# danielbulhosa/CURL

Measured on AMD Instinct MI355X. Metric: Mpix/s through fused curve-apply at 1500x1000 bs32; PSNR delta vs ref, higher is better.
Workload: dtype f32; 1 GPU; CURLLayer.forward fused 3-stage (RGB->Lab->RGB->HSV->RGB + residual), bool mask all ones (every pixel computed); batch_per_gpu=32, global_batch=32, height=1000, width=1500, knots=randn*0.1 (160 per image), parallelism=image-sharded x1, no data-path collective, clock_settle_launches=150

## Files before the change

### curl_amd/csrc/curl_math.h

```cpp
#pragma once
#include <math.h>
#include <type_traits>

#if defined(__HIPCC__)
#define CURL_HD __host__ __device__ __forceinline__
#else
#define CURL_HD inline
#endif

namespace curlm {

CURL_HD float hw_log2(float x) {
#if defined(__HIP_DEVICE_COMPILE__)
  return __builtin_amdgcn_logf(x);
#else
  return log2f(x);
#endif
}
CURL_HD float hw_exp2(float x) {
#if defined(__HIP_DEVICE_COMPILE__)
  return __builtin_amdgcn_exp2f(x);
#else
  return exp2f(x);
#endif
// ... 150 lines not shown
}
template <int M>
CURL_HD void mul_run(float (&y)[M], const float (&a)[M], const float (&b)[M]) {
  for (int i = 0; i < M; ++i) y[i] = a[i] * b[i];
}
template <int M>
CURL_HD void scale_run(float (&y)[M], const float (&a)[M], float k) {
  for (int i = 0; i < M; ++i) y[i] = a[i] * k;
}
template <int M>
CURL_HD void rsub_run(float (&y)[M], float k, const float (&a)[M]) {
  for (int i = 0; i < M; ++i) y[i] = k - a[i];
}
#if defined(__HIP_DEVICE_COMPILE__)
__device__ __forceinline__ float select_le_hw(float x, float thr, float a, float b) {
  unsigned long long m;
  float r;
  asm("v_cmp_le_f32_e64 %0, %1, %2" : "=s"(m) : "v"(x), "s"(thr));
  asm("v_cndmask_b32_e64 %0, %1, %2, %3" : "=v"(r) : "v"(b), "v"(a), "s"(m));
  return r;
}
__device__ __forceinline__ float zero_if_less_hw(float c, float mx, float val) {
  unsigned long long m;
  float r;
  asm("v_cmp_lt_f32_e64 %0, %1, %2" : "=s"(m) : "v"(c), "v"(mx));
  asm("v_cndmask_b32_e64 %0, %1, 0, %2" : "=v"(r) : "v"(val), "s"(m));
  return r;
}
#endif

template <int M>
CURL_HD void select_le_run(float (&out)[M], const float (&x)[M], float thr, const float (&a)[M], const float (&b)[M]) {
#if defined(__HIP_DEVICE_COMPILE__)
#pragma unroll
  for (int i = 0; i < M; ++i) out[i] = select_le_hw(x[i], thr, a[i], b[i]);
  return;
#endif
  float d[M];
  rsub_run(d, thr, x);
#pragma unroll
  for (int i = 0; i < M; ++i) out[i] = blend(neg_mask(d[i]), b[i], a[i]);
}

#if defined(__HIP_DEVICE_COMPILE__)
__device__ __forceinline__ void pred_mul(float& dst, unsigned long long m, float x, float k_uniform) {
  unsigned long long t;
  asm("s_and_saveexec_b64 %1, %2\n\tv_mul_f32_e32 %0, %4, %3\n\ts_mov_b64 exec, %1"
      : "+v"(dst), "=&s"(t) : "s"(m), "v"(x), "s"(k_uniform) : "scc");
}
__device__ __forceinline__ void pred_mul_clamp(float& dst, unsigned long long m, float x, float k_uniform) {
  unsigned long long t;
  asm("s_and_saveexec_b64 %1, %2\n\tv_mul_f32_e64 %0, %4, %3 clamp\n\ts_mov_b64 exec, %1"
      : "+v"(dst), "=&s"(t) : "s"(m), "v"(x), "s"(k_uniform) : "scc");
}
__device__ __forceinline__ void pred_fma(float& dst, unsigned long long m, float x, float k_uniform, float c_vgpr) {
  unsigned long long t;
  asm("s_and_saveexec_b64 %1, %2\n\tv_fma_f32 %0, %3, %4, %5\n\ts_mov_b64 exec, %1"
      : "+v"(dst), "=&s"(t) : "s"(m), "v"(x), "s"(k_uniform), "v"(c_vgpr) : "scc");
}
template <bool BRANCH = true, int M, class A>
__device__ __forceinline__ void select_le_lazy(float (&out)[M], const float (&x)[M], float thr, A a, const float (&b)[M]) {
  unsigned long long m[M], any = BRANCH ? 0ull : 1ull;
#pragma unroll
  for (int i = 0; i < M; ++i) {
    asm("v_cmp_le_f32_e64 %0, %1, %2" : "=s"(m[i]) : "v"(x[i]), "s"(thr));
    if (BRANCH) any |= m[i];
  }
  float r[M];
#pragma unroll
  for (int i = 0; i < M; ++i) r[i] = b[i];
  if (any) {
    if constexpr (std::is_invocable_v<A, float (&)[M], const unsigned long long (&)[M]>) {
      a(r, m);
    } else {
      float av[M];
      a(av);
#pragma unroll
      for (int i = 0; i < M; ++i) asm("v_cndmask_b32_e64 %0, %0, %1, %2" : "+v"(r[i]) : "v"(av[i]), "s"(m[i]));
    }
  }
#pragma unroll
  for (int i = 0; i < M; ++i) out[i] = r[i];
}
#endif

template <int M>
CURL_HD void pow_run(float (&x)[M], float e) {
  CURL_FENCE();
  CURL_TRANS_BEGIN();
#pragma unroll
  for (int i = 0; i < M; ++i) x[i] = hw_log2(x[i]);
  CURL_FENCE();
  scale_run(x, x, e);
  CURL_TRANS_BEGIN();
  CURL_FENCE();
#pragma unroll
  for (int i = 0; i < M; ++i) x[i] = hw_exp2(x[i]);
  CURL_TRANS_END();
  CURL_FENCE();
}

template <int N>
CURL_HD void mat_row(float (&y)[N], const float (&a)[3 * N], float m0, float m1, float m2) {
  for (int i = 0; i < N; ++i) y[i] = fmaf(m2, a[2 * N + i], fmaf(m1, a[N + i], m0 * a[i]));
}

template <int N, int LAZY = 0>
CURL_HD void rgb2lab_n(PxN<N>& p) {
  float x[3 * N], g[3 * N], u2[3 * N], lin[3 * N];
#pragma unroll
  for (int i = 0; i < N; ++i) {
    x[i] = p.c0[i];
    x[N + i] = p.c1[i];
    x[2 * N + i] = p.c2[i];
  }
  fma_run(g, x, kInv1055, (float)(0.055 / 1.055));
  {
    mul_run(u2, g, g);
    pow_run(g, kGammaFrac);
    mul_run(g, u2, g);
  }
#if defined(__HIP_DEVICE_COMPILE__)
  if constexpr (LAZY != 0) {
    const float (&xr)[3 * N] = x;
    select_le_lazy<LAZY == 1>(x, x, kSrgbThr, [&](float (&r)[3 * N], const unsigned long long (&m)[3 * N]) {
#pragma unroll
      for (int i = 0; i < 3 * N; ++i) pred_mul(r[i], m[i], xr[i], kInv1292);
    }, g);
  } else
#endif
  {
    scale_run(lin, x, kInv1292);
    select_le_run(x, x, kSrgbThr, lin, g);
  }
  float t[3 * N], f[3 * N];
  {
    float tx[N], ty[N], tz[N];
    mat_row<N>(tx, x, 0.412453f * kInvXn, 0.357580f * kInvXn, 0.180423f * kInvXn);
    mat_row<N>(ty, x, 0.212671f, 0.715160f, 0.072169f);
    mat_row<N>(tz, x, 0.019334f * kInvZn, 0.119193f * kInvZn, 0.950227f * kInvZn);
#pragma unroll
    for (int i = 0; i < N; ++i) t[i] = tx[i], t[N + i] = ty[i], t[2 * N + i] = tz[i];
  }
#pragma unroll
  for (int i = 0; i < 3 * N; ++i) f[i] = t[i];
  pow_run(f, kThird);
#if defined(__HIP_DEVICE_COMPILE__)
  if constexpr (LAZY != 0) {
    const float (&tr)[3 * N] = t;
    select_le_lazy<LAZY == 1>(f, t, kEps3, [&](float (&r)[3 * N], const unsigned long long (&m)[3 * N]) {
      const float c = k4_29;
#pragma unroll
      for (int i = 0; i < 3 * N; ++i) pred_fma(r[i], m[i], tr[i], kInv3Eps2, c);
    }, f);
  } else
#endif
  {
    fma_run(lin, t, kInv3Eps2, k4_29);
    select_le_run(f, t, kEps3, lin, f);
  }
#pragma unroll
  for (int i = 0; i < N; ++i) {
    float fx = f[i], fy = f[N + i], fz = f[2 * N + i];
    p.c0[i] = fmaf(fy, 1.16f, -0.16f);
    p.c1[i] = fmaf(fx - fy, (float)(500.0 / 220.0), 0.5f);
    p.c2[i] = fmaf(fy - fz, (float)(200.0 / 220.0), 0.5f);
  }
}

template <int N, bool CLAMP12 = false, int LAZY = 0>
CURL_HD void lab2rgb_n(PxN<N>& p) {
  float X[3 * N], v[3 * N], g[3 * N], lin[3 * N];
#pragma unroll
  for (int i = 0; i < N; ++i) {
    float fy = fmaf(p.c0[i], (float)(100.0 / 116.0), (float)(16.0 / 116.0));
    float fx = fmaf(p.c1[i], (float)(220.0 / 500.0), fy - (float)(110.0 / 500.0));
    float fz = fmaf(p.c2[i], (float)(-220.0 / 200.0), fy + (float)(110.0 / 200.0));
    X[i] = fx, X[N + i] = fy, X[2 * N + i] = fz;
  }
  {
    float cub[3 * N];
    mul_run(cub, X, X);
    mul_run(cub, cub, X);
#if defined(__HIP_DEVICE_COMPILE__)
    if constexpr (LAZY != 0) {
      const float (&Xr)[3 * N] = X;
      select_le_lazy<LAZY == 1>(X, X, kEps, [&](float (&r)[3 * N], const unsigned long long (&m)[3 * N]) {
        const float c = -(k3Eps2 * k4_29);
#pragma unroll
        for (int i = 0; i < 3 * N; ++i) pred_fma(r[i], m[i], Xr[i], k3Eps2, c);
      }, cub);
    } else
#endif
    {
      fma_run(lin, X, k3Eps2, -(k3Eps2 * k4_29));
      select_le_run(X, X, kEps, lin, cub);
    }
  }
  {
    float r[N], gg[N], b[N];
    mat_row<N>(r, X, 3.2404542f * kXn, -1.5371385f, -0.4985314f * kZn);
    mat_row<N>(gg, X, -0.9692660f * kXn, 1.8760108f, 0.0415560f * kZn);
    mat_row<N>(b, X, 0.0556434f * kXn, -0.2040259f, 1.0572252f * kZn);
#pragma unroll
    for (int i = 0; i < N; ++i) v[i] = r[i], v[N + i] = gg[i], v[2 * N + i] = b[i];
  }
#pragma unroll
  for (int i = 0; i < 3 * N; ++i) g[i] = v[i];
  pow_run(g, kInvGamma);
  if (!CLAMP12) {
    fma_run(g, g, 1.055f, -0.055f);
#if defined(__HIP_DEVICE_COMPILE__)
    if constexpr (LAZY != 0) {
      const float (&vr)[3 * N] = v;
      select_le_lazy<LAZY == 1>(v, v, kLinThr, [&](float (&r)[3 * N], const unsigned long long (&m)[3 * N]) {
#pragma unroll
        for (int i = 0; i < 3 * N; ++i) pred_mul(r[i], m[i], vr[i], 12.92f);
      }, g);
    } else
#endif
    {
      scale_run(lin, v, 12.92f);
      select_le_run(v, v, kLinThr, lin, g);
    }
  } else {
    float g0[N], v0[N], l0[N], d[3 * N];
#pragma unroll
    for (int i = 0; i < N; ++i) g0[i] = g[i], v0[i] = v[i];
    fma_run(g0, g0, 1.055f, -0.055f);
    scale_run(l0, v0, 12.92f);
    rsub_run(d, kLinThr, v);
#pragma unroll
    for (int i = 0; i < N; ++i) g[i] = g0[i], lin[i] = l0[i];
#if defined(__HIP_DEVICE_COMPILE__)
    if constexpr (LAZY != 0) {
#pragma unroll
      for (int i = N; i < 3 * N; ++i) g[i] = clamp01(fmaf(g[i], 1.055f, -0.055f));
      const float (&vr)[3 * N] = v;
      select_le_lazy<LAZY == 1>(v, v, kLinThr, [&](float (&r)[3 * N], const unsigned long long (&m)[3 * N]) {
#pragma unroll
        for (int i = 0; i < N; ++i) pred_mul(r[i], m[i], vr[i], 12.92f);
#pragma unroll
        for (int i = N; i < 3 * N; ++i) pred_mul_clamp(r[i], m[i], vr[i], 12.92f);
      }, g);
    } else
#endif
    {
#pragma unroll
      for (int i = N; i < 3 * N; ++i) {
        g[i] = clamp01(fmaf(g[i], 1.055f, -0.055f));
        lin[i] = clamp01(v[i] * 12.92f);
      }
#if defined(__HIP_DEVICE_COMPILE__)
#pragma unroll
      for (int i = 0; i < 3 * N; ++i) v[i] = select_le_hw(v[i], kLinThr, lin[i], g[i]);
#else
#pragma unroll
      for (int i = 0; i < 3 * N; ++i) v[i] = blend(neg_mask(d[i]), g[i], lin[i]);
#endif
    }
  }
#pragma unroll
  for (int i = 0; i < N; ++i) {
    p.c0[i] = v[i];
    p.c1[i] = v[N + i];
    p.c2[i] = v[2 * N + i];
  }
}

template <int N, bool UNIT = false>
CURL_HD void rgb2hsv_n(PxN<N>& p) {
  float r[N], g[N], b[N], mx[N], nd[N], rdm[N];
#pragma unroll
  for (int i = 0; i < N; ++i) {
    r[i] = UNIT ? p.c0[i] : clampf(p.c0[i], kHsvFloor, 1.0f);
    g[i] = UNIT ? p.c1[i] : clampf(p.c1[i], kHsvFloor, 1.0f);
    b[i] = UNIT ? p.c2[i] : clampf(p.c2[i], kHsvFloor, 1.0f);
    mx[i] = fmaxf(r[i], fmaxf(g[i], b[i]));
    nd[i] = fminf(r[i], fminf(g[i], b[i])) - mx[i];
    rdm[i] = UNIT ? fmaf(-nd[i], mx[i], 1e-30f) : -nd[i] * mx[i];
  }
  CURL_FENCE();
  CURL_TRANS_BEGIN();
#pragma unroll
  for (int i = 0; i < N; ++i) rdm[i] = UNIT ? hw_rcp(rdm[i]) : rcp_refined(rdm[i]);
  CURL_TRANS_END();
  CURL_FENCE();
#pragma unroll
  for (int i = 0; i < N; ++i) {
    float dfi = rdm[i] * mx[i];
#if defined(__HIP_DEVICE_COMPILE__)
    float t0 = zero_if_less_hw(r[i], mx[i], (g[i] - b[i]) * dfi);
    float t1 = zero_if_less_hw(g[i], mx[i], fmaf(b[i] - r[i], dfi, 2.0f));
    float t2 = zero_if_less_hw(b[i], mx[i], fmaf(r[i] - g[i], dfi, 4.0f));
#else
    float t0 = drop_if(neg_mask(r[i] - mx[i]), (g[i] - b[i]) * dfi);
    float t1 = drop_if(neg_mask(g[i] - mx[i]), fmaf(b[i] - r[i], dfi, 2.0f));
    float t2 = drop_if(neg_mask(b[i] - mx[i]), fmaf(r[i] - g[i], dfi, 4.0f));
#endif
    int live = neg_mask(nd[i]);
    float h = keep_if(live, (t0 + t1) + t2);
    if (UNIT) h = fmaf(h, (float)(1.0 / 6.0), keep_if(neg_mask(h), 1.0f));
    else h = (h + keep_if(neg_mask(h), 6.0f)) * (float)(1.0 / 6.0);
    float s = nd[i] * (rdm[i] * nd[i]);
    if (!UNIT) s = keep_if(live, s);
    p.c0[i] = UNIT ? h : clampf(h, kHsvFloor, 1.0f);
    p.c1[i] = UNIT ? s : clampf(s, kHsvFloor, 1.0f);
    p.c2[i] = UNIT ? mx[i] : clampf(mx[i], kHsvFloor, 1.0f);
  }
}

CURL_HD Px rgb2lab(Px p) {
  PxN<1> q{{p.c0}, {p.c1}, {p.c2}};
  rgb2lab_n<1>(q);
  return Px{q.c0[0], q.c1[0], q.c2[0]};
}
CURL_HD Px lab2rgb(Px p) {
  PxN<1> q{{p.c0}, {p.c1}, {p.c2}};
  lab2rgb_n<1>(q);
  return Px{q.c0[0], q.c1[0], q.c2[0]};
}
CURL_HD Px rgb2hsv(Px p) {
// ... 99 lines not shown
#pragma clang fp contract(off)
#endif
  float sx = S * x;
  float acc0 = 0.0f, acc1 = 0.0f, acc2 = 0.0f;
  int j = 0;
  for (; j + 16 <= n_terms;) {
    for (int e = 0; e < 16; ++e, ++j) {
      float t = sx - (float)j;
      float p = sl[j] * t;
      acc0 = acc0 + p;
    }
    acc1 = acc1 + acc0;
    acc0 = 0.0f;
    if ((j & 0xF0) == 0) {
      acc2 = acc2 + acc1;
      acc1 = 0.0f;
    }
  }
  for (; j < n_terms; ++j) {
    float t = sx - (float)j;
    float p = sl[j] * t;
    acc0 = acc0 + p;
  }
  acc0 = acc0 + acc1;
  acc0 = acc0 + acc2;
  return c0 + acc0;
}

CURL_HD float scale_pwl(float x, const float* C, const float* sl, int K) {
  float sx = (float)(K - 1) * x;
  float fi = clampf(floorf(sx), 0.0f, (float)(K - 2));
  int i = (int)fi;
  float frac = clamp01(sx - fi);
  return fmaf(sl[i], frac, C[i]);
}

CURL_HD float scale_pwl_pairs(float x, const float* tab, int K) {
  float sx = (float)(K - 1) * x;
  float fi = clampf(floorf(sx), 0.0f, (float)(K - 2));
  int i = (int)fi;
  float frac = clamp01(sx - fi);
  return fmaf(tab[2 * i + 1], frac, tab[2 * i]);
}

CURL_HD float scale_exact_pairs(float x, const float* tab, int K) {
#if defined(__clang__)
#pragma clang fp contract(off)
#endif
  const int n_terms = K - 2;
  const float sx = (float)(K - 1) * x;
  float acc0 = 0.0f, acc1 = 0.0f, acc2 = 0.0f;
  int j = 0;
  for (; j + 16 <= n_terms;) {
    for (int e = 0; e < 16; ++e, ++j) {
      float t = sx - (float)j;
      float p = tab[2 * j + 1] * t;
      acc0 = acc0 + p;
    }
    acc1 = acc1 + acc0;
    acc0 = 0.0f;
    if ((j & 0xF0) == 0) {
      acc2 = acc2 + acc1;
      acc1 = 0.0f;
    }
  }
  for (; j < n_terms; ++j) {
    float t = sx - (float)j;
    float p = tab[2 * j + 1] * t;
    acc0 = acc0 + p;
  }
  acc0 = acc0 + acc1;
  acc0 = acc0 + acc2;
  return tab[0] + acc0;
}
template <int MODE>
CURL_HD float scale_tab(float x, const float* tab, int K) {
  return MODE == 1 ? scale_exact_pairs(x, tab, K) : scale_pwl_pairs(x, tab, K);
}

struct LayerCoef {
  Affine lab[3], rgb[3], hsv[4];
};

template <bool BINARY, int N, bool CLAMP12 = false>
CURL_HD void lab_stage_n(PxN<N>& p, const float (&m)[N], const Affine* k) {
  rgb2lab_n<N, 1>(p);
#pragma unroll
  for (int i = 0; i < N; ++i) {
    Px o = adjust3(Px{p.c0[i], p.c1[i], p.c2[i]}, k[0], k[1], k[2]);
    if (!BINARY) {
      o.c0 *= m[i];
      o.c1 *= m[i];
      o.c2 *= m[i];
    }
    p.c0[i] = o.c0, p.c1[i] = o.c1, p.c2[i] = o.c2;
  }
  lab2rgb_n<N, CLAMP12, 1>(p);
}
CURL_HD Px lab_stage_masked_out() { return lab2rgb(Px{0.0f, 0.0f, 0.0f}); }

template <bool BINARY, int N>
CURL_HD void hsv_stage_n(PxN<N>& p, const float (&m)[N], const Affine* k) {
  rgb2hsv_n<N>(p);
#pragma unroll
  for (int i = 0; i < N; ++i) {
    Px h = adjust_hsv4(Px{p.c0[i], p.c1[i], p.c2[i]}, k[0], k[1], k[2], k[3]);
    if (!BINARY) {
      h.c0 *= m[i];
      h.c1 *= m[i];
      h.c2 *= m[i];
    }
    Px o = hsv2rgb<BINARY>(h);
    if (BINARY) {
      o.c0 *= m[i];
      o.c1 *= m[i];
      o.c2 *= m[i];
    }
    p.c0[i] = o.c0, p.c1[i] = o.c1, p.c2[i] = o.c2;
  }
}

template <bool BINARY, int N>
CURL_HD void curl_layer_n(PxN<N>& p, const float (&m)[N], const LayerCoef& k) {
  PxN<N> in = p;
  lab_stage_n<BINARY, N, true>(p, m, k.lab);
#pragma unroll
  for (int i = 0; i < N; ++i) {
    Px o = adjust3<true>(Px{p.c0[i], p.c1[i], p.c2[i]}, k.rgb[0], k.rgb[1], k.rgb[2]);
    if (!BINARY) {
      o.c0 *= m[i];
      o.c1 *= m[i];
      o.c2 *= m[i];
    }
    p.c0[i] = o.c0, p.c1[i] = o.c1, p.c2[i] = o.c2;
  }
  rgb2hsv_n<N, BINARY>(p);
#pragma unroll
  for (int i = 0; i < N; ++i) {
    Px h = adjust_hsv4<BINARY>(Px{p.c0[i], p.c1[i], p.c2[i]}, k.hsv[0], k.hsv[1], k.hsv[2], k.hsv[3]);
    if (!BINARY) {
      h.c0 *= m[i];
      h.c1 *= m[i];
      h.c2 *= m[i];
    }
    Px res = hsv2rgb<BINARY>(h);
    p.c0[i] = clamp01(in.c0[i] + res.c0) * m[i];
    p.c1[i] = clamp01(in.c1[i] + res.c1) * m[i];
    p.c2[i] = clamp01(in.c2[i] + res.c2) * m[i];
  }
}

template <bool BINARY>
CURL_HD Px lab_stage(Px in, float m, const Affine* k) {
  PxN<1> q{{in.c0}, {in.c1}, {in.c2}};
  const float mm[1] = {m};
  lab_stage_n<BINARY, 1>(q, mm, k);
  return Px{q.c0[0], q.c1[0], q.c2[0]};
}
template <bool BINARY>
CURL_HD Px hsv_stage(Px in, float m, const Affine* k) {
  PxN<1> q{{in.c0}, {in.c1}, {in.c2}};
  const float mm[1] = {m};
  hsv_stage_n<BINARY, 1>(q, mm, k);
  return Px{q.c0[0], q.c1[0], q.c2[0]};
}
template <bool BINARY>
CURL_HD Px curl_layer(Px in, float m, const LayerCoef& k) {
  PxN<1> q{{in.c0}, {in.c1}, {in.c2}};
  const float mm[1] = {m};
  curl_layer_n<BINARY, 1>(q, mm, k);
  return Px{q.c0[0], q.c1[0], q.c2[0]};
}

}
```

### curl_amd/csrc/kernels/host_api.inc

```
static int check_img(const void* in, const void* out, int B, int H, int W) {
  if (!in || !out) return fail(CURL_E_NULL, "image pointer is NULL");
  if (B <= 0 || H <= 0 || W <= 0) return fail(CURL_E_SHAPE, "B, H, W must be positive");
  if ((uint64_t)H * (uint64_t)W > (1ull << 30)) return fail(CURL_E_SHAPE, "H*W exceeds 2^30 pixels");
  if (B > 65535) return fail(CURL_E_SHAPE, "B exceeds 65535 images per call");
  return 0;
}
static int check_coeffs_aligned(const float* coeffs, int num_coeffs) {
  if (num_coeffs == 126 && (uintptr_t)coeffs % 8) return fail(CURL_E_SHAPE, "coeffs must be 8-byte aligned (num_coeffs = 126)");
  if ((uintptr_t)coeffs % 4) return fail(CURL_E_SHAPE, "coeffs must be 4-byte aligned");
  return 0;
}
static int check_flags(unsigned flags, unsigned allowed) {
  const unsigned tune = CURL_F_TUNE_UNROLL_MASK | CURL_F_TUNE_BLOCK_MASK | CURL_F_TUNE_XCD_MASK | CURL_F_TUNE_OCC_MASK | CURL_F_TUNE_PREP_MASK | CURL_F_MASK_FIRST | CURL_F_TUNE_NO_NT | CURL_F_DIAG_NO_MEM;
  if (flags & ~(allowed | tune)) return fail(CURL_E_FLAGS, "unsupported flag bit for this entry point");
  if ((flags & CURL_F_EXACT_ORDER) && (flags & CURL_F_PWL))
    return fail(CURL_E_FLAGS, "CURL_F_EXACT_ORDER and CURL_F_PWL are exclusive");
  if (((flags & CURL_F_TUNE_PREP_MASK) >> CURL_F_TUNE_PREP_SHIFT) > 2)
    return fail(CURL_E_FLAGS, "curve-collapse placement must be 0 (library's choice), 1 (separate launch) or 2 (in the kernel)");
  return 0;
}

static bool planes_vec4(size_t HW, const void* mask, int mask_kind, const void* p0, const void* p1 = nullptr,
                        const void* p2 = nullptr, const void* p3 = nullptr) {
  bool ok = (HW % 4 == 0) && (((uintptr_t)p0 | (uintptr_t)p1 | (uintptr_t)p2 | (uintptr_t)p3) % 16 == 0);
  if (mask_kind == CURL_MASK_F32 && ((uintptr_t)mask % 16)) ok = false;
  if (mask_kind == CURL_MASK_U8 && ((uintptr_t)mask % 4)) ok = false;
  return ok;
}
#define DISPATCH_VEC_MASK(LAUNCH, aligned, mask_kind, ...)                            \
  do {                                                                                \
    if (aligned) {                                                                    \
      if ((mask_kind) == CURL_MASK_U8) LAUNCH(4, CURL_MASK_U8, ##__VA_ARGS__);        \
      else if ((mask_kind) == CURL_MASK_F32) LAUNCH(4, CURL_MASK_F32, ##__VA_ARGS__); \
      else LAUNCH(4, CURL_MASK_NONE, ##__VA_ARGS__);                                  \
    } else {                                                                          \
      if ((mask_kind) == CURL_MASK_U8) LAUNCH(1, CURL_MASK_U8, ##__VA_ARGS__);        \
      else if ((mask_kind) == CURL_MASK_F32) LAUNCH(1, CURL_MASK_F32, ##__VA_ARGS__); \
      else LAUNCH(1, CURL_MASK_NONE, ##__VA_ARGS__);                                  \
    }                                                                                 \
  } while (0)

constexpr unsigned kXcdDefault = 1;
struct Geometry {
  int xcd = 0;
  int vec;
  int unroll;
  unsigned n;
  unsigned blocks_per_image, n_blocks, n_images;
  int nt;
  unsigned threads = 256;
  unsigned units = 0, segs = 0;
  unsigned lds_cap = 0;
};
static int make_row_geometry(Geometry& g, int B, int H, int W) {
  if (g.vec == 4 && W % 4 != 0) g.vec = 1;
  g.units = (unsigned)(W / g.vec);
  unsigned best_t = 64, best_waste = ~0u;
  for (unsigned t = 64; t <= 256; t += 64) {
    unsigned segs = (g.units + t - 1) / t, waste = segs * t - g.units;
    if (waste <= best_waste) best_waste = waste, best_t = t;
  }
  g.threads = best_t;
  g.segs = (g.units + best_t - 1) / best_t;
  g.n = (unsigned)((size_t)H * W / g.vec);
  uint64_t per_image = (uint64_t)g.segs * (uint64_t)H;
  if (per_image * (uint64_t)B > 0x7fffffffull || per_image > 0x7fffffffull) return fail(CURL_E_SHAPE, "grid too large");
  g.blocks_per_image = (unsigned)per_image;
  g.n_blocks = (unsigned)(per_image * (uint64_t)B);
  return 0;
}


static unsigned lds_for_resident(unsigned k, unsigned static_bytes = 0) {
  const unsigned total = (k == 2 ? 43u : 128u / k) * 1280u;
  return total > static_bytes ? total - static_bytes : 0u;
}
template <auto Kernel>
static unsigned static_lds() {
  static const unsigned v = [] {
    hipFuncAttributes a;
    return hipFuncGetAttributes(&a, reinterpret_cast<const void*>(Kernel)) == hipSuccess ? (unsigned)a.sharedSizeBytes : 0u;
  }();
  return v;
}
constexpr unsigned kResidentMinTiles = 5632u;
constexpr unsigned kResPsnr = 3, kResEgress = 4, kResIngress = 4, kResLoss = 0, kResLossBwd = 0;
static unsigned aux_lds(unsigned k_resident, const dim3& grid, bool float4_path, unsigned static_bytes) {
  return (k_resident > 1 && float4_path && (uint64_t)grid.x * grid.y >= kResidentMinTiles) ? lds_for_resident(k_resident, static_bytes) : 0u;
}

static int make_geometry(Geometry& g, const void* p0, const void* p1, const void* pm, int mask_kind, int B, int H, int W,
                         unsigned flags, int default_unroll, size_t also_multiple_of_4 = 0) {
  size_t HW = (size_t)H * W;
  bool aligned = (HW % 4 == 0) && (also_multiple_of_4 % 4 == 0) && (((uintptr_t)p0 | (uintptr_t)p1) % 16 == 0);
  if (pm && mask_kind == CURL_MASK_F32 && ((uintptr_t)pm % 16)) aligned = false;
  if (pm && mask_kind == CURL_MASK_U8 && ((uintptr_t)pm % 4)) aligned = false;
  g.vec = aligned ? 4 : 1;
  int u = (int)((flags & CURL_F_TUNE_UNROLL_MASK) >> CURL_F_TUNE_UNROLL_SHIFT);
  if (u == 0) u = default_unroll;
  if (u != 1 && u != 2 && u != 4) return fail(CURL_E_FLAGS, "tuning unroll must be 1, 2 or 4");
  g.unroll = u;
  g.n = (unsigned)(HW / g.vec);
  const unsigned bsel = (flags & CURL_F_TUNE_BLOCK_MASK) >> CURL_F_TUNE_BLOCK_SHIFT;
  if (bsel > 2) return fail(CURL_E_FLAGS, "tuning block size must be 0 (256), 1 (128) or 2 (64 threads)");
  g.threads = 256u >> bsel;
  unsigned per_chunk = g.threads * (unsigned)u;
  g.blocks_per_image = (g.n + per_chunk - 1) / per_chunk;
  uint64_t nb = (uint64_t)g.blocks_per_image * (uint64_t)B;
  if (nb > 0x7fffffffull) return fail(CURL_E_SHAPE, "grid too large");
  g.n_blocks = (unsigned)nb;
  g.nt = (flags & CURL_F_TUNE_NO_NT) ? 0 : 1;
  g.n_images = (unsigned)B;
  unsigned xsel = (flags & CURL_F_TUNE_XCD_MASK) >> CURL_F_TUNE_XCD_SHIFT;
  if (xsel > 2) return fail(CURL_E_FLAGS, "tuning tile mapping must be 0 (default), 1 (plain) or 2 (XCD-contiguous)");
  g.xcd = (xsel ? xsel : kXcdDefault) == 2;
  const unsigned occ = (flags & CURL_F_TUNE_OCC_MASK) >> CURL_F_TUNE_OCC_SHIFT;
  g.lds_cap = occ > 1 ? lds_for_resident(occ) : 0u;
  return 0;
}

template <class Op, int VEC, int MK, bool NT>
static hipError_t launch_u(const Geometry& g, const StreamArgs& a, hipStream_t s) {
  dim3 grid(a.xcd_per ? 8u * a.xcd_per : g.blocks_per_image, g.n_images), block(g.threads);
  if constexpr (Op::kSingleTileShape) {
    hipLaunchKernelGGL((stream_kernel<Op, VEC, 1, MK, NT>), grid, block, g.lds_cap, s, a);
  } else {
    switch (g.unroll) {
      case 1:
        if constexpr (Op::kMask && MK == CURL_MASK_U8 && VEC == 4 && NT && Op::kLdsFloats == 0) {
          if (a.mask_first == 1) {
            hipLaunchKernelGGL((stream_kernel<Op, VEC, 1, MK, NT, FMT_F32CHW, true>), grid, block, g.lds_cap, s, a);
            break;
          }
        }
        hipLaunchKernelGGL((stream_kernel<Op, VEC, 1, MK, NT>), grid, block, g.lds_cap, s, a);
        break;
      case 2:
        hipLaunchKernelGGL((stream_kernel<Op, VEC, 2, MK, NT>), grid, block, g.lds_cap, s, a);
        break;
      default:
        hipLaunchKernelGGL((stream_kernel<Op, VEC, 4, MK, NT>), grid, block, g.lds_cap, s, a);
        break;
    }
  }
  return hipGetLastError();
}

template <class Op, int MK>
static hipError_t launch_v(const Geometry& g, const StreamArgs& a, hipStream_t s) {
  if (g.vec == 4) return g.nt ? launch_u<Op, 4, MK, true>(g, a, s) : launch_u<Op, 4, MK, false>(g, a, s);
  return launch_u<Op, 1, MK, false>(g, a, s);
}

static PrepArgs make_prep(const float* r0, int n0, int K0, const float* r1, int n1, int K1, const float* r2, int n2, int K2,
                          float* ws, unsigned stride, float* reg) {
  PrepArgs p;
  p.raw[0] = r0, p.raw[1] = r1, p.raw[2] = r2;
  p.ncurves[0] = n0, p.ncurves[1] = n1, p.ncurves[2] = n2;
  p.K[0] = K0, p.K[1] = K1, p.K[2] = K2;
  p.ws = ws;
  p.reg_out = reg;
  p.stride = stride;
  return p;
}
static int launch_prep(const PrepArgs& p, int B, hipStream_t s) {
  hipLaunchKernelGGL(knots_prep_kernel, dim3(B), dim3(256), 0, s, p);
  hipError_t e = hipGetLastError();
  if (e != hipSuccess) return hip_fail(e, "knots_prep_kernel");
  return 0;
}
static int run_prep(const float* r0, int n0, int K0, const float* r1, int n1, int K1, const float* r2, int n2, int K2,
                    float* ws, unsigned stride, float* reg, int B, hipStream_t s) {
  return launch_prep(make_prep(r0, n0, K0, r1, n1, K1, r2, n2, K2, ws, stride, reg), B, s);
}

struct Slab {
  int H_full = 0, row0 = 0;
};

constexpr unsigned kSelfPrepMaxTiles = 2048u;

template <class Op, int MK>
static hipError_t launch_selfprep(const Geometry& g, const StreamArgs& a, const PrepArgs& p, hipStream_t s) {
  dim3 grid(g.blocks_per_image, g.n_images), block(256);
  if (g.vec == 4) hipLaunchKernelGGL((stream_selfprep_kernel<Op, 4, MK, true>), grid, block, 0, s, a, p);
  else hipLaunchKernelGGL((stream_selfprep_kernel<Op, 1, MK, false>), grid, block, 0, s, a, p);
  return hipGetLastError();
}

template <class Op>
static int launch_stream(const float* in, float* out, const void* mask, int mask_kind, const float* coef,
                         unsigned coef_stride, int B, int H, int W, unsigned flags, hipStream_t s, const char* name,
                         int op_flag = 0, Slab slab = Slab(), const PrepArgs* prep = nullptr) {
  Geometry g;
  bool self_prep = false;
  if (prep) {
    if constexpr (Op::kSelfPrep) {
      const unsigned psel = (flags & CURL_F_TUNE_PREP_MASK) >> CURL_F_TUNE_PREP_SHIFT;
      const unsigned shape = CURL_F_TUNE_UNROLL_MASK | CURL_F_TUNE_BLOCK_MASK | CURL_F_TUNE_XCD_MASK | CURL_F_TUNE_OCC_MASK |
                             CURL_F_TUNE_NO_NT | CURL_F_DIAG_NO_MEM | CURL_F_MASK_FIRST;
      Geometry probe;
      const size_t ppx = slab.H_full ? (size_t)slab.H_full * W : (size_t)H * W;
      if (int rc = make_geometry(probe, in, out, mask, mask_kind, B, H, W, 1u << CURL_F_TUNE_UNROLL_SHIFT, 1, ppx | (size_t)slab.row0 * W))
        return rc;
      self_prep = !(flags & shape) && !Op::kMaskFirst && (psel == 2 || (psel == 0 && probe.n_blocks <= kSelfPrepMaxTiles));
    }
    if (!self_prep)
      if (int rc = launch_prep(*prep, B, s)) return rc;
  }
  flags &= ~CURL_F_TUNE_PREP_MASK;
  if (self_prep) flags |= 1u << CURL_F_TUNE_UNROLL_SHIFT;

  if (Op::kSingleTileShape) flags &= ~CURL_F_TUNE_UNROLL_MASK;
  const size_t plane_px = slab.H_full ? (size_t)slab.H_full * W : (size_t)H * W, off_px = (size_t)slab.row0 * W;
// ... 1127 lines not shown
```

### curl_amd/csrc/kernels/ops.inc

```
struct NoK {};
struct OpDefaults {
  static constexpr bool kSingleTileShape = false;
  static constexpr int kLdsFloats = 0;
  static constexpr int kMinWavesPerSimd = 1;
  static constexpr bool kRowTiles = false;
  static constexpr bool kStageValue = false;
  static constexpr int kRawFloats = 0;
  static constexpr int kResident = 0;
  static constexpr bool kMaskFirst = false;
  static constexpr bool kSelfPrep = false;
};
#define CONVERTER_OP(NAME, FN, RES)                                                      \
  struct NAME : OpDefaults {                                                             \
    typedef NoK K;                                                                       \
    static constexpr bool kMask = false;                                                 \
    static constexpr int kUnroll = 2;                                                    \
    static constexpr int kResident = RES;                                                \
    static __device__ __forceinline__ K load(const float*, const StreamArgs&) { return K{}; } \
    template <bool, int N>                                                               \
    static __device__ __forceinline__ void apply_n(PxN<N>& p, const float (&)[N], const K&, unsigned) { FN(p); } \
    static constexpr bool kBlendMaskedOut = false;                                       \
    static __device__ __forceinline__ Px masked_out(const K&) { return Px{0.0f, 0.0f, 0.0f}; } \
  };
CONVERTER_OP(OpRgb2Lab, rgb2lab_n<N>, 4)
// ... 83 lines not shown
  struct K {
    Affine k[4];
  };
  static constexpr bool kMask = true;
  static constexpr int kUnroll = 2;
  static constexpr int kResident = 4;
  static __device__ __forceinline__ K load(const float* ws, const StreamArgs&) {
    K k;
#pragma unroll
    for (int c = 0; c < 4; ++c) k.k[c] = load_affine(ws, c);
    return k;
  }
  template <bool BINARY, int N>
  static __device__ __forceinline__ void apply_n(PxN<N>& p, const float (&m)[N], const K& k, unsigned) {
    hsv_stage_n<BINARY, N>(p, m, k.k);
  }
  static constexpr bool kBlendMaskedOut = false;
  static __device__ __forceinline__ Px masked_out(const K&) { return Px{0.0f, 0.0f, 0.0f}; }
};
template <int MODE>
struct OpLabStageTab : OpDefaults {
  struct K {
    const float* tab;
    int n;
    Px masked;
  };
  static constexpr bool kMask = true;
  static constexpr int kUnroll = 1;
  static constexpr bool kSingleTileShape = true;
  static constexpr bool kStageValue = true;
  static constexpr int kLdsFloats = 6 * CURL_MAX_KNOTS + 4;
  static __device__ __forceinline__ unsigned lds_count(const StreamArgs& a) { return 6u * (unsigned)a.op_flag + 3u; }
  static __device__ __forceinline__ float stage_value(const float* ws, unsigned i, unsigned, const StreamArgs& a) {
    const unsigned Kn = (unsigned)a.op_flag, n6 = 6u * Kn;
    if (i >= n6) return ws[WS_MASKED + (i - n6)];
    unsigned j = i >> 1, jj = j % Kn;
    float c = ws[WS_KNOTS + j];
    if ((i & 1u) == 0u) return c;
    return (jj + 1u < Kn) ? ws[WS_KNOTS + j + 1u] - c : 0.0f;
  }
  static __device__ __forceinline__ K load(const float* lds, const StreamArgs& a) {
    const int n6 = 6 * a.op_flag;
    return K{lds, a.op_flag, Px{lds[n6], lds[n6 + 1], lds[n6 + 2]}};
  }
  template <bool BINARY, int N>
  static __device__ __forceinline__ void apply_n(PxN<N>& p, const float (&m)[N], const K& k, unsigned) {
    rgb2lab_n<N>(p);
    const float* T = k.tab;
#pragma unroll
    for (int i = 0; i < N; ++i) {
      float c0 = clamp01(p.c0[i] * scale_tab<MODE>(p.c0[i], T, k.n));
      float c1 = clamp01(p.c1[i]), c2 = clamp01(p.c2[i]);
      c1 = clamp01(c1 * scale_tab<MODE>(c1, T + 2 * k.n, k.n));
      c2 = clamp01(c2 * scale_tab<MODE>(c2, T + 4 * k.n, k.n));
      if (!BINARY) c0 *= m[i], c1 *= m[i], c2 *= m[i];
      p.c0[i] = c0, p.c1[i] = c1, p.c2[i] = c2;
    }
    lab2rgb_n<N>(p);
  }
  static constexpr bool kBlendMaskedOut = true;
  static __device__ __forceinline__ Px masked_out(const K& k) { return k.masked; }
};
struct OpLayer : OpDefaults {
  static constexpr bool kSelfPrep = true;
  typedef LayerCoef K;
  static constexpr bool kMask = true;
  static constexpr int kUnroll = 1;
  static __device__ __forceinline__ K load(const float* ws, const StreamArgs&) {
    K k;
#pragma unroll
    for (int c = 0; c < 3; ++c) k.lab[c] = load_affine(ws, c);
#pragma unroll
    for (int c = 0; c < 3; ++c) k.rgb[c] = load_affine(ws, 3 + c);
#pragma unroll
    for (int c = 0; c < 4; ++c) k.hsv[c] = load_affine(ws, 6 + c);
    return k;
  }
  template <bool BINARY, int N>
  static __device__ __forceinline__ void apply_n(PxN<N>& p, const float (&m)[N], const K& k, unsigned) {
    curl_layer_n<BINARY, N>(p, m, k);
  }
  static constexpr bool kBlendMaskedOut = false;
  static __device__ __forceinline__ Px masked_out(const K&) { return Px{0.0f, 0.0f, 0.0f}; }
};

template <int MODE>
struct OpLayerTab : OpDefaults {
  struct K {
    const float* tab;
    int kl, kr, kh;
  };
  static constexpr bool kMask = true;
  static constexpr int kUnroll = 1;
  static constexpr bool kSingleTileShape = true;
  static constexpr bool kStageValue = true;
  static constexpr int kLdsFloats = 2 * MAX_CURVES * CURL_MAX_KNOTS;
  static __device__ __forceinline__ int n_knots(int f) { return 3 * (f & 1023) + 3 * ((f >> 10) & 1023) + 4 * (f >> 20); }
  static __device__ __forceinline__ unsigned lds_count(const StreamArgs& a) { return 2u * (unsigned)n_knots(a.op_flag); }
  static __device__ __forceinline__ float stage_value(const float* ws, unsigned i, unsigned, const StreamArgs& a) {
    const int f = a.op_flag;
    const unsigned kl = f & 1023, kr = (f >> 10) & 1023, kh = f >> 20, j = i >> 1;
    float c = ws[WS_KNOTS + j];
    if ((i & 1u) == 0u) return c;
    unsigned in_curve = j < 3u * kl ? j % kl : j < 3u * kl + 3u * kr ? (j - 3u * kl) % kr : (j - 3u * kl - 3u * kr) % kh;
    unsigned Kc = j < 3u * kl ? kl : j < 3u * kl + 3u * kr ? kr : kh;
    return (in_curve + 1u < Kc) ? ws[WS_KNOTS + j + 1u] - c : 0.0f;
  }
  static __device__ __forceinline__ K load(const float* lds, const StreamArgs& a) {
    const int f = a.op_flag;
    return K{lds, f & 1023, (f >> 10) & 1023, f >> 20};
  }
  static __device__ __forceinline__ Px adjust3_pwl(Px p, const float* T, int Kc) {
    Px o;
    o.c0 = clamp01(p.c0 * scale_tab<MODE>(p.c0, T, Kc));
    float c1 = clamp01(p.c1), c2 = clamp01(p.c2);
    o.c1 = clamp01(c1 * scale_tab<MODE>(c1, T + 2 * Kc, Kc));
    o.c2 = clamp01(c2 * scale_tab<MODE>(c2, T + 4 * Kc, Kc));
    return o;
  }
  template <bool BINARY, int N>
  static __device__ __forceinline__ void apply_n(PxN<N>& p, const float (&m)[N], const K& k, unsigned) {
    const PxN<N> in = p;
    const float *Tl = k.tab, *Tr = k.tab + 6 * k.kl, *Th = Tr + 6 * k.kr;
    rgb2lab_n<N>(p);
#pragma unroll
    for (int i = 0; i < N; ++i) {
      Px o = adjust3_pwl(Px{p.c0[i], p.c1[i], p.c2[i]}, Tl, k.kl);
      p.c0[i] = o.c0 * m[i], p.c1[i] = o.c1 * m[i], p.c2[i] = o.c2 * m[i];
    }
    lab2rgb_n<N>(p);
#pragma unroll
    for (int i = 0; i < N; ++i) {
      Px o = adjust3_pwl(Px{p.c0[i], p.c1[i], p.c2[i]}, Tr, k.kr);
      p.c0[i] = o.c0 * m[i], p.c1[i] = o.c1 * m[i], p.c2[i] = o.c2 * m[i];
    }
    rgb2hsv_n<N>(p);
#pragma unroll
    for (int i = 0; i < N; ++i) {
      float h = clamp01(p.c0[i] * scale_tab<MODE>(p.c0[i], Th, k.kh));
      float sc = clamp01(p.c1[i]), vc = clamp01(p.c2[i]);
      sc = clamp01(sc * scale_tab<MODE>(h, Th + 2 * k.kh, k.kh));
      sc = clamp01(sc * scale_tab<MODE>(sc, Th + 4 * k.kh, k.kh));
      vc = clamp01(vc * scale_tab<MODE>(vc, Th + 6 * k.kh, k.kh));
      Px res = hsv2rgb(Px{h * m[i], sc * m[i], vc * m[i]});
      p.c0[i] = clamp01(in.c0[i] + res.c0) * m[i];
      p.c1[i] = clamp01(in.c1[i] + res.c1) * m[i];
      p.c2[i] = clamp01(in.c2[i] + res.c2) * m[i];
    }
  }
  static constexpr bool kBlendMaskedOut = false;
  static __device__ __forceinline__ Px masked_out(const K&) { return Px{0.0f, 0.0f, 0.0f}; }
};

template <int V>
struct OpTriSpace : OpDefaults {
  struct K {
    const float* coef;
    unsigned W;
    float fW, fH;
    bool residual_only;
  };
  static constexpr bool kMask = false;
  static constexpr int kUnroll = 1;
  static constexpr bool kSingleTileShape = true;
  static constexpr int kLdsFloats = 9 * PolyEval<V>::kSeqStride;
  static constexpr int kMinWavesPerSimd = kTriSpaceWaves;
// ... 103 lines not shown
```

### curl_amd/csrc/kernels/stream.inc

```
typedef float v4f __attribute__((ext_vector_type(4)));
typedef unsigned v4b;

struct StreamArgs {
  const float* in;
  float* out;
  const void* mask;
  const float* coef;
  unsigned coef_stride;
  unsigned n;
  unsigned blocks_per_image;
  unsigned n_blocks;
  int no_mem;
  unsigned W, H;
  int op_flag;
  int mask_first;
  const uint8_t* white;
  unsigned units, segs;
  unsigned plane, off, row0;
  unsigned xcd_per;
};
#define FMT_F32CHW 0
#define FMT_U8HWC 1

template <int VEC>
// ... 251 lines not shown
  const unsigned img = blockIdx.y;
  unsigned chunk = blockIdx.x;
  if (!Op::kRowTiles && a.xcd_per) {
    chunk = (blockIdx.x & 7u) * a.xcd_per + (blockIdx.x >> 3);
    if (chunk >= a.blocks_per_image) return;
  }
  __builtin_assume(a.n <= (1u << 28));
  const float* table = a.coef ? a.coef + (size_t)img * a.coef_stride : nullptr;
  __shared__ __attribute__((aligned(16))) float s_table[Op::kLdsFloats > 0 ? Op::kLdsFloats : 1];
  unsigned row = 0, base = chunk * (blockDim.x * U) + threadIdx.x;
  bool valid = true;
  if constexpr (Op::kRowTiles) {
    row = chunk / a.segs;
    const unsigned in_row = (chunk - row * a.segs) * blockDim.x + threadIdx.x;
    valid = in_row < a.units;
    base = row * a.units + min(in_row, a.units - 1u);
  }
  const size_t plane = (size_t)a.plane;
  const size_t image_bytes = (FMT == FMT_U8HWC) ? 3 * plane * VEC : 3 * plane * sizeof(T);
  const size_t slab_bytes = (FMT == FMT_U8HWC) ? 3 * (size_t)a.off * VEC : (size_t)a.off * sizeof(T);
  const T* p0 = reinterpret_cast<const T*>(reinterpret_cast<const char*>(a.in) + (size_t)img * image_bytes + slab_bytes);
  T* q0 = reinterpret_cast<T*>(reinterpret_cast<char*>(a.out) + (size_t)img * image_bytes + slab_bytes);
  const size_t mask_off = (size_t)img * plane + a.off;
  Tile<VEC, U, MK> t;
  constexpr bool kEarlyLoads = Op::kLdsFloats > 0 && FMT == FMT_F32CHW;
  if constexpr (kEarlyLoads) load_tile<VEC, U, MK, NT, FMT>(t, a, p0, plane, mask_off, base);
  if constexpr (Op::kLdsFloats > 0) {
    if constexpr (Op::kRawFloats > 0) {
      typedef float f2 __attribute__((ext_vector_type(2)));
      static_assert(Op::kRawFloats % 2 == 0, "copied as 8-byte pairs");
      __shared__ __attribute__((aligned(16))) float s_raw[(Op::kRawFloats + 3) & ~3];
      constexpr unsigned n2 = Op::kRawFloats / 2;
      const f2* g = reinterpret_cast<const f2*>(table);
      for (unsigned i0 = 0; i0 < n2; i0 += 4u * blockDim.x) {
        f2 r[4];
#pragma unroll
        for (unsigned k = 0; k < 4; ++k) r[k] = g[min(i0 + k * blockDim.x + threadIdx.x, n2 - 1u)];
#pragma unroll
        for (unsigned k = 0; k < 4; ++k) {
          const unsigned i = i0 + k * blockDim.x + threadIdx.x;
          if (i < n2) reinterpret_cast<f2*>(s_raw)[i] = r[k];
        }
      }
      __syncthreads();
      table = s_raw;
    }
    if constexpr (Op::kRowTiles || Op::kStageValue) {
      const unsigned n_stage = Op::lds_count(a);
      for (unsigned i = threadIdx.x; i < n_stage; i += blockDim.x)
        s_table[i] = Op::stage_value(table, i, row + a.row0, a);
    } else {
      for (int i = threadIdx.x; i < Op::kLdsFloats; i += blockDim.x) s_table[i] = table[Op::stage_index(i)];
    }
    __syncthreads();
    table = s_table;
  }
  const typename Op::K k = Op::load(table, a);
  static_assert(!MASK_FIRST || (U == 1 && MK == CURL_MASK_U8 && VEC == 4 && FMT == FMT_F32CHW && Op::kMask && !kEarlyLoads),
                "the mask-first variant exists for bool / uint8 masks on the float4 kernels at one group per lane");
  bool pixels_asked_for = false;
  if constexpr (MASK_FIRST) {
    {
      typedef typename Pack<VEC>::M M;
      const unsigned i = min(base, a.n - 1u);
      t.mb[0] = ld<NT>(reinterpret_cast<const M*>(reinterpret_cast<const char*>(reinterpret_cast<const M*>(a.mask) + mask_off) +
                                                   i * (unsigned)sizeof(M)));
      if (__builtin_amdgcn_ballot_w64(t.mb[0] != 0u) == 0ull) {
        if (base < a.n && valid) {
          const Px z = Op::masked_out(k);
          const unsigned boff = base * (unsigned)sizeof(T);
          st<NT>(reinterpret_cast<T*>(reinterpret_cast<char*>(q0) + boff), T(z.c0));
          st<NT>(reinterpret_cast<T*>(reinterpret_cast<char*>(q0 + plane) + boff), T(z.c1));
          st<NT>(reinterpret_cast<T*>(reinterpret_cast<char*>(q0 + 2 * plane) + boff), T(z.c2));
        }
        return;
      }
      load_tile<VEC, U, MK, NT, FMT, true>(t, a, p0, plane, mask_off, base);
      pixels_asked_for = true;
    }
  }
  if constexpr (!kEarlyLoads)
    if (!pixels_asked_for) load_tile<VEC, U, MK, NT, FMT>(t, a, p0, plane, mask_off, base);
  compute_store<Op, VEC, U, MK, NT, FMT>(t, a, q0, plane, base, k, valid);
}

template <class K>
__device__ __forceinline__ K uniform_k(K k) {
  static_assert(sizeof(K) % 4 == 0 && std::is_trivially_copyable<K>::value, "a struct of floats");
  unsigned w[sizeof(K) / 4];
  __builtin_memcpy(w, &k, sizeof(K));
#pragma unroll
  for (unsigned i = 0; i < sizeof(K) / 4; ++i) w[i] = __builtin_amdgcn_readfirstlane(w[i]);
  __builtin_memcpy(&k, w, sizeof(K));
  return k;
}

template <class Op, int VEC, int MK, bool NT>
__global__ __launch_bounds__(256, Op::kMinWavesPerSimd) void stream_selfprep_kernel(StreamArgs a, PrepArgs p) {
  typedef typename Pack<VEC>::T T;
  static_assert(Op::kLdsFloats == 0 && !Op::kRowTiles && Op::kSelfPrep, "ops whose per-image table is the workspace row's head");
  const unsigned img = blockIdx.y, chunk = blockIdx.x;
  __builtin_assume(a.n <= (1u << 28));
  __builtin_assume(a.no_mem == 0);
  const unsigned base = chunk * blockDim.x + threadIdx.x;
  const size_t plane = (size_t)a.plane;
  const size_t image_bytes = 3 * plane * sizeof(T), slab_bytes = (size_t)a.off * sizeof(T);
  const T* p0 = reinterpret_cast<const T*>(reinterpret_cast<const char*>(a.in) + (size_t)img * image_bytes + slab_bytes);
  T* q0 = reinterpret_cast<T*>(reinterpret_cast<char*>(a.out) + (size_t)img * image_bytes + slab_bytes);
  const size_t mask_off = (size_t)img * plane + a.off;
  Tile<VEC, 1, MK> t;
  float first_raw = prep_fetch_first(p, img);
  __builtin_amdgcn_sched_barrier(0);
  load_tile<VEC, 1, MK, NT, FMT_F32CHW>(t, a, p0, plane, mask_off, base);
  __shared__ float s_head[WS_KNOTS];
  prep_image(p, img, chunk == 0, s_head, first_raw, true);
  __syncthreads();
  const typename Op::K k = uniform_k(Op::load(s_head, a));
  compute_store<Op, VEC, 1, MK, NT, FMT_F32CHW>(t, a, q0, plane, base, k, true);
}
```

Measured before the change: 240,400 Mpix/s.

## Add per-pixel lazy Lab branch and a lean dedicated kernel for the layer op

Adds a LAZY==3 mode where the rgb2lab cube-root linear-segment fixup is skipped per pixel slot (across all three channels) when no lane needs it, instead of one wave-wide any-check. A new OpLayerLarge uses this mode and runs through a stripped-down stream_layer_large_kernel that assumes memory is live and skips the validity and early-mask paths. The host dispatches to it by default for u8 masks with VEC=4, non-temporal stores and 256 threads. Possible costs are extra branch overhead and loss of the generic kernel's early-mask skipping, which does not apply here since the mask is all ones.

```diff
diff --git a/curl_amd/csrc/curl_math.h b/curl_amd/csrc/curl_math.h
--- a/curl_amd/csrc/curl_math.h
+++ b/curl_amd/csrc/curl_math.h
@@ -256,6 +256,33 @@
 #pragma unroll
   for (int i = 0; i < M; ++i) out[i] = r[i];
 }
+template <int M, class A>
+__device__ __forceinline__ void select_le_lazy_slots(float (&out)[M], const float (&x)[M], float thr, float c, A a,
+                                                     const float (&b)[M]) {
+  static_assert(M % 3 == 0, "three planes of N values");
+  constexpr int N = M / 3;
+  unsigned long long m[M], any = 0ull;
+#pragma unroll
+  for (int i = 0; i < M; ++i) {
+    asm("v_cmp_le_f32_e64 %0, %1, %2" : "=s"(m[i]) : "v"(x[i]), "s"(thr));
+    any |= m[i];
+  }
+  float r[M];
+#pragma unroll
+  for (int i = 0; i < M; ++i) r[i] = b[i];
+  if (any) {
+    asm volatile("" : "+v"(c));
+#pragma unroll
+    for (int e = 0; e < N; ++e) {
+      if (m[e] | m[N + e] | m[2 * N + e]) {
+#pragma unroll
+        for (int ch = 0; ch < 3; ++ch) a(r, m, ch * N + e, c);
+      }
+    }
+  }
+#pragma unroll
+  for (int i = 0; i < M; ++i) out[i] = r[i];
+}
 #endif
 
 template <int M>
@@ -297,7 +324,7 @@
 #if defined(__HIP_DEVICE_COMPILE__)
   if constexpr (LAZY != 0) {
     const float (&xr)[3 * N] = x;
-    select_le_lazy<LAZY == 1>(x, x, kSrgbThr, [&](float (&r)[3 * N], const unsigned long long (&m)[3 * N]) {
+    select_le_lazy<LAZY == 1 || LAZY == 3>(x, x, kSrgbThr, [&](float (&r)[3 * N], const unsigned long long (&m)[3 * N]) {
 #pragma unroll
       for (int i = 0; i < 3 * N; ++i) pred_mul(r[i], m[i], xr[i], kInv1292);
     }, g);
@@ -320,7 +347,12 @@
   for (int i = 0; i < 3 * N; ++i) f[i] = t[i];
   pow_run(f, kThird);
 #if defined(__HIP_DEVICE_COMPILE__)
-  if constexpr (LAZY != 0) {
+  if constexpr (LAZY == 3) {
+    const float (&tr)[3 * N] = t;
+    select_le_lazy_slots(f, t, kEps3, k4_29, [&](float (&r)[3 * N], const unsigned long long (&m)[3 * N], int i, float c) {
+      pred_fma(r[i], m[i], tr[i], kInv3Eps2, c);
+    }, f);
+  } else if constexpr (LAZY != 0) {
     const float (&tr)[3 * N] = t;
     select_le_lazy<LAZY == 1>(f, t, kEps3, [&](float (&r)[3 * N], const unsigned long long (&m)[3 * N]) {
       const float c = k4_29;
@@ -387,7 +419,7 @@
 #if defined(__HIP_DEVICE_COMPILE__)
     if constexpr (LAZY != 0) {
       const float (&vr)[3 * N] = v;
-      select_le_lazy<LAZY == 1>(v, v, kLinThr, [&](float (&r)[3 * N], const unsigned long long (&m)[3 * N]) {
+      select_le_lazy<LAZY == 1 || LAZY == 3>(v, v, kLinThr, [&](float (&r)[3 * N], const unsigned long long (&m)[3 * N]) {
 #pragma unroll
         for (int i = 0; i < 3 * N; ++i) pred_mul(r[i], m[i], vr[i], 12.92f);
       }, g);
@@ -411,7 +443,7 @@
 #pragma unroll
       for (int i = N; i < 3 * N; ++i) g[i] = clamp01(fmaf(g[i], 1.055f, -0.055f));
       const float (&vr)[3 * N] = v;
-      select_le_lazy<LAZY == 1>(v, v, kLinThr, [&](float (&r)[3 * N], const unsigned long long (&m)[3 * N]) {
+      select_le_lazy<LAZY == 1 || LAZY == 3>(v, v, kLinThr, [&](float (&r)[3 * N], const unsigned long long (&m)[3 * N]) {
 #pragma unroll
         for (int i = 0; i < N; ++i) pred_mul(r[i], m[i], vr[i], 12.92f);
 #pragma unroll
@@ -677,9 +709,9 @@
   Affine lab[3], rgb[3], hsv[4];
 };
 
-template <bool BINARY, int N, bool CLAMP12 = false>
+template <bool BINARY, int N, bool CLAMP12 = false, int LAZY = 1>
 CURL_HD void lab_stage_n(PxN<N>& p, const float (&m)[N], const Affine* k) {
-  rgb2lab_n<N, 1>(p);
+  rgb2lab_n<N, LAZY>(p);
 #pragma unroll
   for (int i = 0; i < N; ++i) {
     Px o = adjust3(Px{p.c0[i], p.c1[i], p.c2[i]}, k[0], k[1], k[2]);
@@ -690,7 +722,7 @@
     }
     p.c0[i] = o.c0, p.c1[i] = o.c1, p.c2[i] = o.c2;
   }
-  lab2rgb_n<N, CLAMP12, 1>(p);
+  lab2rgb_n<N, CLAMP12, LAZY>(p);
 }
 CURL_HD Px lab_stage_masked_out() { return lab2rgb(Px{0.0f, 0.0f, 0.0f}); }
 
@@ -715,10 +747,10 @@
   }
 }
 
-template <bool BINARY, int N>
+template <bool BINARY, int N, int LAZY = 1>
 CURL_HD void curl_layer_n(PxN<N>& p, const float (&m)[N], const LayerCoef& k) {
   PxN<N> in = p;
-  lab_stage_n<BINARY, N, true>(p, m, k.lab);
+  lab_stage_n<BINARY, N, true, LAZY>(p, m, k.lab);
 #pragma unroll
   for (int i = 0; i < N; ++i) {
     Px o = adjust3<true>(Px{p.c0[i], p.c1[i], p.c2[i]}, k.rgb[0], k.rgb[1], k.rgb[2]);
diff --git a/curl_amd/csrc/kernels/host_api.inc b/curl_amd/csrc/kernels/host_api.inc
--- a/curl_amd/csrc/kernels/host_api.inc
+++ b/curl_amd/csrc/kernels/host_api.inc
@@ -43,6 +43,7 @@
 constexpr unsigned kXcdDefault = 1;
 struct Geometry {
   int xcd = 0;
+  bool xcd_asked = false;
   int vec;
   int unroll;
   unsigned n;
@@ -114,6 +115,7 @@
   unsigned xsel = (flags & CURL_F_TUNE_XCD_MASK) >> CURL_F_TUNE_XCD_SHIFT;
   if (xsel > 2) return fail(CURL_E_FLAGS, "tuning tile mapping must be 0 (default), 1 (plain) or 2 (XCD-contiguous)");
   g.xcd = (xsel ? xsel : kXcdDefault) == 2;
+  g.xcd_asked = xsel != 0;
   const unsigned occ = (flags & CURL_F_TUNE_OCC_MASK) >> CURL_F_TUNE_OCC_SHIFT;
   g.lds_cap = occ > 1 ? lds_for_resident(occ) : 0u;
   return 0;
@@ -130,6 +132,12 @@
         if constexpr (Op::kMask && MK == CURL_MASK_U8 && VEC == 4 && NT && Op::kLdsFloats == 0) {
           if (a.mask_first == 1) {
             hipLaunchKernelGGL((stream_kernel<Op, VEC, 1, MK, NT, FMT_F32CHW, true>), grid, block, g.lds_cap, s, a);
+            break;
+          }
+        }
+        if constexpr (std::is_same<Op, OpLayer>::value && MK == CURL_MASK_U8 && VEC == 4 && NT) {
+          if (!g.xcd_asked && g.threads == 256u && !a.no_mem) {
+            hipLaunchKernelGGL((stream_layer_large_kernel<OpLayerLarge>), grid, block, g.lds_cap, s, a);
             break;
           }
         }
diff --git a/curl_amd/csrc/kernels/ops.inc b/curl_amd/csrc/kernels/ops.inc
--- a/curl_amd/csrc/kernels/ops.inc
+++ b/curl_amd/csrc/kernels/ops.inc
@@ -189,6 +189,12 @@
   }
   static constexpr bool kBlendMaskedOut = false;
   static __device__ __forceinline__ Px masked_out(const K&) { return Px{0.0f, 0.0f, 0.0f}; }
+};
+struct OpLayerLarge : OpLayer {
+  template <bool BINARY, int N>
+  static __device__ __forceinline__ void apply_n(PxN<N>& p, const float (&m)[N], const K& k, unsigned) {
+    curl_layer_n<BINARY, N, 3>(p, m, k);
+  }
 };
 
 template <int MODE>
diff --git a/curl_amd/csrc/kernels/stream.inc b/curl_amd/csrc/kernels/stream.inc
--- a/curl_amd/csrc/kernels/stream.inc
+++ b/curl_amd/csrc/kernels/stream.inc
@@ -357,6 +357,25 @@
   if constexpr (!kEarlyLoads)
     if (!pixels_asked_for) load_tile<VEC, U, MK, NT, FMT>(t, a, p0, plane, mask_off, base);
   compute_store<Op, VEC, U, MK, NT, FMT>(t, a, q0, plane, base, k, valid);
+}
+
+template <class Op>
+__global__ __launch_bounds__(256, Op::kMinWavesPerSimd) void stream_layer_large_kernel(StreamArgs a) {
+  typedef typename Pack<4>::T T;
+  static_assert(Op::kLdsFloats == 0 && !Op::kRowTiles && Op::kMask, "a masked op whose per-image table is read through scalar loads");
+  const unsigned img = blockIdx.y, chunk = blockIdx.x;
+  __builtin_assume(a.n <= (1u << 28));
+  __builtin_assume(a.no_mem == 0);
+  const unsigned base = chunk * blockDim.x + threadIdx.x;
+  const size_t plane = (size_t)a.plane;
+  const size_t image_bytes = 3 * plane * sizeof(T), slab_bytes = (size_t)a.off * sizeof(T);
+  const T* p0 = reinterpret_cast<const T*>(reinterpret_cast<const char*>(a.in) + (size_t)img * image_bytes + slab_bytes);
+  T* q0 = reinterpret_cast<T*>(reinterpret_cast<char*>(a.out) + (size_t)img * image_bytes + slab_bytes);
+  const size_t mask_off = (size_t)img * plane + a.off;
+  Tile<4, 1, CURL_MASK_U8> t;
+  const typename Op::K k = Op::load(a.coef + (size_t)img * a.coef_stride, a);
+  load_tile<4, 1, CURL_MASK_U8, true, FMT_F32CHW>(t, a, p0, plane, mask_off, base);
+  compute_store<Op, 4, 1, CURL_MASK_U8, true, FMT_F32CHW>(t, a, q0, plane, base, k, true);
 }
 
 template <class K>
```

Result: no change. 241,200 Mpix/s (median of 6 runs) (+0.3%).
